# Nemo157/regex

Measured on AMD Instinct MI355X. Metric: haystack GB/s scanned + matches/s, batched bytes::Regex::find, 1/2/4/8 MI355X, higher is better.
Workload: dtype u8; 1 GPU; C2: find \d{4}-\d{2}-\d{2} over 1048576 x 4096 B haystacks per GPU; haystacks_per_gpu=1048576, haystack_bytes=4096, parallelism=dp1

## Files before the change

include/rure_amd.h:

```cpp
#ifndef RURE_AMD_H
#define RURE_AMD_H

#include <stdbool.h>
#include <stddef.h>
#include <stdint.h>

#ifdef __cplusplus
extern "C" {
#endif


typedef struct rure rure;
typedef struct rure_set rure_set;
typedef struct rure_options rure_options;
typedef struct rure_iter rure_iter;
typedef struct rure_error rure_error;
typedef struct rure_captures rure_captures;
typedef struct rure_iter_capture_names rure_iter_capture_names;

#define RURE_FLAG_CASEI (1 << 0)
#define RURE_FLAG_MULTI (1 << 1)
#define RURE_FLAG_DOTNL (1 << 2)
#define RURE_FLAG_SWAP_GREED (1 << 3)
#define RURE_FLAG_SPACE (1 << 4)
// ... 229 lines not shown
  RURE_AMD_PATH_ITER_CHUNKED = -21,
  RURE_AMD_PATH_ITER_WAVE = -22,
  RURE_AMD_PATH_REPLACE_CLASS = -23,
  RURE_AMD_PATH_REPLACE_HMAP = -24,
  RURE_AMD_PATH_ITER_SHADOW_GATED = -25,
  RURE_AMD_PATH_ITER_WAVE_SERVED = -27,
  RURE_AMD_PATH_CAPTURES_ITER = -28,
  RURE_AMD_PATH_REPLACE_EXPAND = -29
} rure_amd_path;
int rure_amd_last_fwd_path(void);
uint64_t rure_amd_last_iter_units(uint64_t *haystacks);
uint64_t rure_amd_last_long_units(uint64_t *haystacks, uint64_t *chunk);
uint64_t rure_amd_last_set_units(uint64_t *haystacks, uint64_t *chunk);
uint64_t rure_amd_last_lazy_long(uint64_t *haystacks, uint64_t *chunk, uint32_t *rounds, uint32_t *fell_back);
typedef struct rure_amd_tile_skip {
  int32_t eligible;
  int32_t m;
  int32_t anchor_a, anchor_b;
  int32_t used;
} rure_amd_tile_skip;
int rure_amd_tile_skip_info(rure *re, rure_amd_tile_skip *info);
int64_t rure_amd_tile_skip_simulate(rure *re, const uint8_t *hay, size_t len, uint32_t *states_skip,
                                    uint32_t *states_exact, uint8_t *dirty);
int rure_amd_debug_set(const char *spec);
int rure_amd_kernel_timer(int on);
double rure_amd_kernel_timer_read(uint64_t *launches);

#ifdef __cplusplus
}
#endif
#endif
```

regex_amd/__init__.py:

```python
import ctypes

from . import _native as N

__all__ = ["Regex", "RegexSet", "Error", "NoExpand", "NONE", "Path", "release_scratch"]

NONE = N.NONE
Path = N.Path


def _ser_lits(lits):
    out = bytearray()
    for v, cut in lits:
        out += bytes([1 if cut else 0]) + len(v).to_bytes(4, "little") + bytes(v)
    return bytes(out)


def _de_lits(buf):
    out, i = [], 0
    while i < len(buf):
        cut, n = buf[i] != 0, int.from_bytes(buf[i + 1:i + 5], "little")
        out.append((bytes(buf[i + 5:i + 5 + n]), cut))
        i += 5 + n
    return out

# ... 615 lines not shown
    def dfa_info(self, which=0):
        info = N.DfaInfo()
        rc = N.rure_amd_dfa_info_get(self._re, which, ctypes.byref(info))
        return {k: getattr(info, k) for k, _ in N.DfaInfo._fields_} if rc == N.OK else None

    def tile_skip_info(self):
        info = N.TileSkipInfo()
        rc = N.rure_amd_tile_skip_info(self._re, ctypes.byref(info))
        return {k: getattr(info, k) for k, _ in N.TileSkipInfo._fields_} if rc == N.OK else None

    def tile_skip_simulate(self, hay):
        import numpy as np
        hay = np.ascontiguousarray(np.frombuffer(bytes(hay), dtype=np.uint8))
        n = len(hay) // 128
        ss = np.zeros(max(n, 1), dtype=np.uint32)
        se = np.zeros(max(n, 1), dtype=np.uint32)
        d = np.zeros(max(n, 1), dtype=np.uint8)
        rc = N.rure_amd_tile_skip_simulate(self._re, hay.ctypes.data, len(hay), ss.ctypes.data, se.ctypes.data,
                                           d.ctypes.data)
        if rc < 0:
            return None
        return ss[:n], se[:n], d[:n]

    def first_bytes(self):
        buf = (ctypes.c_uint8 * 4)()
        n = N.rure_amd_first_byte_export(self._re, buf)
        return bytes(buf[:n]) if n > 0 else None

    def lex_table(self, ascii=False):
        import numpy as np
        if ascii:
            ex = lambda t, n, s: N.rure_amd_lex_ascii_export(self._re, 0, t, n, s)
        else:
            ex = lambda t, n, s: N.rure_amd_lex_export(self._re, t, n, s)
        n = ex(None, 0, None)
        if n <= 0:
            return None
        t = np.zeros(n, dtype=np.uint8)
        s0 = ctypes.c_uint32()
        ex(t.ctypes.data, n, ctypes.byref(s0))
        return t, s0.value

    def run_class(self, ascii=False):
        import numpy as np
        c = np.zeros(256, dtype=np.uint8)
        return c if N.rure_amd_run_class_export(self._re, 1 if ascii else 0, c.ctypes.data) == 1 else None
# ... 393 lines not shown
```

regex_amd/_native.py:

```python
import ctypes
import enum
import os

_HERE = os.path.dirname(os.path.abspath(__file__))
LIB_PATH = os.path.join(_HERE, "lib", "librure_amd.so")
if os.environ.get("RURE_AMD_LIB_AB"):
    LIB_PATH = os.path.join(_HERE, "lib", os.path.basename(os.environ["RURE_AMD_LIB_AB"]))

if not os.path.exists(LIB_PATH):
    raise ImportError(
        "regex_amd: native library %s is missing; build it with `make` or "
        "`python -c 'import __graft_entry__ as g; g.build()'`" % LIB_PATH)

try:
    import torch
except ImportError:
    pass

lib = ctypes.CDLL(LIB_PATH)

c_u8p = ctypes.POINTER(ctypes.c_uint8)
c_size = ctypes.c_size_t


# ... 167 lines not shown

def last_iter_units():
    n = ctypes.c_uint64(0)
    units = rure_amd_last_iter_units(ctypes.byref(n))
    return int(units), int(n.value)


rure_amd_last_long_units = _sig("rure_amd_last_long_units", ctypes.c_uint64, ctypes.POINTER(ctypes.c_uint64),
                                ctypes.POINTER(ctypes.c_uint64))


def last_long_units():
    n, c = ctypes.c_uint64(0), ctypes.c_uint64(0)
    units = rure_amd_last_long_units(ctypes.byref(n), ctypes.byref(c))
    return int(units), int(n.value), int(c.value)


class TileSkipInfo(ctypes.Structure):
    _fields_ = [(n, ctypes.c_int32) for n in ("eligible", "m", "anchor_a", "anchor_b", "used")]


rure_amd_tile_skip_info = _sig("rure_amd_tile_skip_info", ctypes.c_int, VP, ctypes.POINTER(TileSkipInfo))
rure_amd_tile_skip_simulate = _sig("rure_amd_tile_skip_simulate", ctypes.c_int64, VP, VP, c_size, VP, VP, VP)
rure_amd_last_set_units = _sig("rure_amd_last_set_units", ctypes.c_uint64, ctypes.POINTER(ctypes.c_uint64),
                               ctypes.POINTER(ctypes.c_uint64))
rure_amd_set_long_dfa_export = _sig("rure_amd_set_long_dfa_export", ctypes.c_int, VP, ctypes.POINTER(DfaInfo), VP, VP,
                                    VP, VP, VP, VP)
class LazyInfo(ctypes.Structure):
    _fields_ = [(k, ctypes.c_uint32) for k in ("states", "columns", "rows_built", "hot_rows", "rounds", "fell_back")]


rure_amd_set_lazy_export = _sig("rure_amd_set_lazy_export", ctypes.c_int, VP, ctypes.POINTER(LazyInfo), VP, VP, VP,
                                VP, VP, VP)
rure_amd_set_lazy_build = _sig("rure_amd_set_lazy_build", ctypes.c_int, VP, VP, c_size, c_size)
rure_amd_lazy_export = _sig("rure_amd_lazy_export", ctypes.c_int, VP, ctypes.POINTER(LazyInfo), VP, VP, VP, VP, VP)
rure_amd_lazy_build = _sig("rure_amd_lazy_build", ctypes.c_int, VP, VP, c_size, c_size)
rure_amd_lazy_strip_export = _sig("rure_amd_lazy_strip_export", ctypes.c_int, VP, VP)
rure_amd_set_lazy_strip_export = _sig("rure_amd_set_lazy_strip_export", ctypes.c_int, VP, VP, VP)
rure_amd_set_lazy_strip_build = _sig("rure_amd_set_lazy_strip_build", ctypes.c_int, VP, VP, c_size)
rure_amd_lazy_strip_build = _sig("rure_amd_lazy_strip_build", ctypes.c_int, VP, VP, c_size)
rure_amd_last_lazy_long = _sig("rure_amd_last_lazy_long", ctypes.c_uint64, ctypes.POINTER(ctypes.c_uint64),
                               ctypes.POINTER(ctypes.c_uint64), ctypes.POINTER(ctypes.c_uint32),
                               ctypes.POINTER(ctypes.c_uint32))
rure_amd_debug_set = _sig("rure_amd_debug_set", ctypes.c_int, ctypes.c_char_p)
rure_amd_first_byte_export = _sig("rure_amd_first_byte_export", ctypes.c_int, VP, VP)
rure_amd_lex_export = _sig("rure_amd_lex_export", ctypes.c_int64, VP, VP, c_size, VP)
# ... 46 lines not shown
```

regex_amd/csrc/capi.cpp:

```cpp
#include "runtime.hpp"
#include "host/chain_map.hpp"
#include "host/expand.hpp"

namespace {


void fill_prog_info(const Program &p, rure_amd_prog_info *info) {
  info->ninsts = (uint32_t)p.insts.size();
  info->start = p.start;
  info->nmatches = (uint32_t)p.matches.size();
  info->ncaptures = (uint32_t)p.capture_names.size();
  info->anchored_start = p.anchored_start;
  info->anchored_end = p.anchored_end;
  info->has_unicode_word_boundary = p.has_unicode_word_boundary;
  info->is_reverse = p.is_reverse;
  memcpy(info->byte_classes, p.byte_classes, 256);
}

int64_t export_prog(const Program &p, rure_amd_prog_info *info, rure_amd_inst *insts, size_t cap) {
  if (info) fill_prog_info(p, info);
  if (insts) {
    size_t n = std::min(cap, p.insts.size());
    for (size_t i = 0; i < n; ++i) {
      const Inst &in = p.insts[i];
// ... 1205 lines not shown
}
int rure_amd_tile_skip_info(rure *re, rure_amd_tile_skip *info) {
  if (!re || !info) return RURE_AMD_ERR_ARG;
  memset(info, 0, sizeof(*info));
  if (!build_regex(re) || !re->dfa_ok) return RURE_AMD_ERR_DFA;
  const TileSkip &k = re->tskip;
  info->eligible = k.ok ? 1 : 0;
  info->used = k.ok && k.use ? 1 : 0;
  info->m = (int32_t)k.m;
  info->anchor_a = k.ok ? (int32_t)k.pa : -1;
  info->anchor_b = k.ok ? (int32_t)k.pb : -1;
  return RURE_AMD_OK;
}

int64_t rure_amd_tile_skip_simulate(rure *re, const uint8_t *hay, size_t len, uint32_t *states_skip,
                                    uint32_t *states_exact, uint8_t *dirty) {
  if (!re || (!hay && len) || !states_skip || !states_exact || !dirty) return RURE_AMD_ERR_ARG;
  if (!build_regex(re) || !re->dfa_ok) return RURE_AMD_ERR_DFA;
  if (!re->tskip.ok) return RURE_AMD_ERR_ARG;
  return (int64_t)tile_skip_simulate(re->tskip, re->pf.lds.data(), re->pf.hot, re->pf.full.data(),
                                     (uint32_t)re->dfwd.n_match_end, hay, len, states_skip, states_exact, dirty);
}

int rure_amd_debug_set(const char *spec) { return rure_amd::knob_set(spec) ? RURE_AMD_OK : RURE_AMD_ERR_ARG; }



int64_t rure_amd_literals_syntax(const uint8_t *pattern, size_t length, uint32_t flags, int which, size_t limit_size,
                                 size_t limit_class, uint8_t *out, size_t cap) {
  Expr e;
  std::string err;
  if (!parse_regex(std::string((const char *)pattern, length), syntax_flags(flags), &e, &err)) return RURE_AMD_ERR_ARG;
  Literals l;
  l.limit_size = limit_size;
  l.limit_class = limit_class;
  if (which == 0) l.union_prefixes(e);
  else l.union_suffixes(e);
  std::string o;
  ser_lits(l.lits, &o);
  return put_out(o, out, cap);
}

int64_t rure_amd_literals_op(int op, const uint8_t *in, size_t in_len, uint8_t *out, size_t cap) {
  Literals l;
  if ((in_len && !in) || !de_lits(in, in_len, &l.lits)) return RURE_AMD_ERR_ARG;
  std::string o;
// ... 56 lines not shown
```

regex_amd/csrc/host/tile_skip.cpp:

```cpp
#include "tile_skip.hpp"

#include <algorithm>
#include <cstring>
#include <set>
#include <unordered_set>

#include "../kernels/dfa_scan.hpp"
#include "byte_freq.h"

namespace rure_amd {

namespace {

constexpr uint32_t kMaxPos = 16;

AsciiSet from_cranges(const std::vector<CRange> &r) {
  AsciiSet s;
  for (const CRange &x : r)
    for (uint32_t c = x.lo; c <= x.hi && c < 128; ++c) s.add(c);
  return s;
}

AsciiSet from_branges(const std::vector<BRange> &r) {
  AsciiSet s;
// ... 88 lines not shown
void tile_skip_analyse(const Expr &e, const uint8_t *lds, uint32_t hot, uint32_t ustart1, TileSkip *out) {
  TileSkip k;
  auto fail = [&](const std::string &w) { k.ok = false; k.why = w; *out = k; };
  if (!tile_skip_sequence(e, &k.seq, &k.why)) return fail(k.why);
  const uint32_t m = k.m = (uint32_t)k.seq.size();
  for (uint32_t b = 0; b < 128; ++b)
    for (uint32_t j = 0; j < m; ++j)
      if (k.seq[j].has(b)) k.sa[b] |= (uint16_t)(1u << j);
  struct Cand { double p; uint32_t pos; uint8_t lo, hi; };
  std::vector<Cand> cs;
  for (uint32_t j = 0; j < m; ++j) {
    uint8_t lo, hi;
    if (single_range(k.seq[j], &lo, &hi)) cs.push_back({range_freq(lo, hi), j, lo, hi});
  }
  if (cs.empty()) return fail("no position is a single byte range");
  std::stable_sort(cs.begin(), cs.end(), [](const Cand &x, const Cand &y) { return x.p < y.p; });
  Cand a = cs[0], b = cs.size() > 1 ? cs[1] : cs[0];
  if (a.pos > b.pos) std::swap(a, b);
  const double rate = 128.0 * a.p * (a.pos == b.pos ? 1.0 : b.p);
  if (rate >= 1.0) return fail("the anchors are too frequent");
  k.use = 64.0 * rate < 1.0;
  k.pa = a.pos; k.pb = b.pos;
  k.a_lo = a.lo; k.a_hi = a.hi; k.b_lo = b.lo; k.b_hi = b.hi;
  if (hot == 0 || hot > 63) return fail("no hot table of at most 63 rows");
  if (!ustart1) return fail("(S) the start state depends on the flags");
  k.s0 = ustart1 - 1;
  if (k.s0 >= hot) return fail("(S) the start state is not hot");
  auto step = [&](uint32_t s, uint32_t c) { return (uint32_t)lds[(size_t)s * kRow + c]; };
  const uint32_t fin = 1u << (m - 1);
  constexpr size_t kMaxProduct = 1 << 15;
  std::unordered_set<uint32_t> seen;
  std::vector<uint32_t> work;
  seen.insert(k.s0 << 17);
  work.push_back(k.s0 << 17);
  while (!work.empty()) {
    const uint32_t key = work.back(), s = key >> 17, D = (key >> 1) & 0xFFFFu, pc = key & 1u;
    work.pop_back();
    k.reach |= 1ull << s;
    for (uint32_t c = 0; c < 128; ++c) {
      const uint32_t D2 = ((D << 1) | 1u) & k.sa[c];
      const uint32_t comp = (D2 & fin) ? 1u : 0u;
      const uint32_t t = step(s, c);
      if (t == hot) {
        if (!comp && !pc) return fail("(A) the hot rows are left without a window of the sequence");
        continue;
      }
// ... 13 lines not shown
      for (uint32_t c = 0; c < 128; ++c) {
        const uint32_t p2 = step(pq.first, c);
        if (p2 == hot) continue;
        const uint32_t q2 = step(pq.second, c);
        if (q2 == hot) return fail("(B) the run from the start state leaves the hot rows first");
        next.insert({p2, q2});
      }
    level.swap(next);
  }
  for (const auto &pq : level)
    if (pq.first != pq.second) return fail("(B) the state after 16 bytes depends on the state before them");
  k.ok = true;
  *out = k;
}

void tile_skip_dev(const TileSkip &k, const uint16_t *sa, TileSkipDev *out) {
  TileSkipDev d{};
  const uint32_t rep = 0x01010101u;
  d.on = k.use ? 1 : 0; d.m = k.m; d.pa = k.pa; d.pb = k.pb; d.s0 = k.s0; d.reach = k.reach;
  d.gt_a = (0x7Fu - k.a_hi) * rep; d.lt_a = (0x7Fu + k.a_lo) * rep;
  d.gt_b = (0x7Fu - k.b_hi) * rep; d.lt_b = (0x7Fu + k.b_lo) * rep;
  d.eq_a = k.a_lo * rep; d.eq_b = k.b_lo * rep;
  d.single = k.a_lo == k.a_hi && k.b_lo == k.b_hi;
  d.sa = sa;
  *out = d;
}

namespace {

struct HostSrc {
  const uint8_t *p;
  uint4 row(int r) const {
    uint4 v;
    memcpy(&v, p + 16 * r, 16);
    return v;
  }
  uint32_t byte(uint32_t i) const { return p[i]; }
};

}

size_t tile_skip_simulate(const TileSkip &k, const uint8_t *lds, uint32_t hot, const uint16_t *full,
                          uint32_t n_match_end, const uint8_t *hay, size_t len, uint32_t *states_skip,
                          uint32_t *states_exact, uint8_t *dirty) {
  TileSkipDev kd;
  tile_skip_dev(k, k.sa, &kd);
// ... 12 lines not shown
    if (!done) {
      if (!d) {
        uint32_t c = k.s0;
        for (int j = 112; j < 128; ++j) c = lds[(size_t)c * kRow + p[j]];
        s = c;
        ln.prev_dirty = 0;
      } else {
        bool left = s >= hot;
        for (int j = 0; j < 128 && !done; ++j) {
          s = full[(size_t)s * 256 + p[j]];
          left = left || s >= hot;
          done = over(s);
        }
        ln.prev_dirty = (f & kSkipOwn) || left;
      }
    }
    states_skip[t] = s;
    for (int j = 0; j < 128 && !over(x); ++j) x = full[(size_t)x * 256 + p[j]];
    states_exact[t] = x;
  }
  return ntiles;
}

}
```

regex_amd/csrc/host/tile_skip.hpp:

```cpp
#pragma once
#include <cstdint>
#include <string>
#include <vector>

#include "syntax.hpp"

namespace rure_amd {

struct AsciiSet {
  uint64_t w[2] = {0, 0};
  bool has(uint32_t b) const { return (w[b >> 6] >> (b & 63)) & 1; }
  void add(uint32_t b) { w[b >> 6] |= 1ull << (b & 63); }
  bool empty() const { return !(w[0] | w[1]); }
};

struct TileSkip {
  bool ok = false;
  bool use = false;
  std::string why;
  uint32_t m = 0;
  std::vector<AsciiSet> seq;
  uint32_t pa = 0, pb = 0;
  uint8_t a_lo = 0, a_hi = 0, b_lo = 0, b_hi = 0;
  uint32_t s0 = 0;
  uint64_t reach = 0;
  uint16_t sa[128] = {0};
};

struct TileSkipDev;
void tile_skip_dev(const TileSkip &k, const uint16_t *sa, TileSkipDev *out);

bool tile_skip_sequence(const Expr &e, std::vector<AsciiSet> *seq, std::string *why);

void tile_skip_analyse(const Expr &e, const uint8_t *lds, uint32_t hot, uint32_t ustart1, TileSkip *out);

size_t tile_skip_simulate(const TileSkip &k, const uint8_t *lds, uint32_t hot, const uint16_t *full,
                          uint32_t n_match_end, const uint8_t *hay, size_t len, uint32_t *states_skip,
                          uint32_t *states_exact, uint8_t *dirty);

}
```

regex_amd/csrc/kernels/dfa_scan.hip:

```cpp
#include <hip/hip_runtime.h>
#include <stdint.h>

#include <algorithm>
#include <cstdlib>
#include <mutex>
#include <vector>

#include "dfa_device.hpp"

namespace rure_amd {

__device__ __forceinline__ void note_quit(uint32_t *flag) {
  if (flag) atomicOr(flag, 1u);
}

template <int MODE>
__device__ __forceinline__ void finish_lane(const LaneState &L, const RevDfaDev &r, const uint8_t *base,
                                            uint64_t len, uint64_t lo, uint64_t h, void *out, uint32_t *qf,
                                            const uint8_t *rlds = nullptr) {
  if (L.quit) note_quit(qf);
  if (MODE == MODE_ISMATCH) {
    ((uint8_t *)out)[h] = L.quit ? 2 : (L.last != NONE ? 1 : 0);
    return;
  }
// ... 176 lines not shown
  const bool strided = b.offs == nullptr;
  if (!strided && b.defer)
    return mode == MODE_FIND ? launch_lit_find_m<MODE_FIND, false, true>(b, f, out, st, grid)
                             : launch_lit_find_m<MODE_ISMATCH, false, true>(b, f, out, st, grid);
  if (mode == MODE_FIND)
    return strided ? launch_lit_find_m<MODE_FIND, true>(b, f, out, st, grid)
                   : launch_lit_find_m<MODE_FIND, false>(b, f, out, st, grid);
  return strided ? launch_lit_find_m<MODE_ISMATCH, true>(b, f, out, st, grid)
                 : launch_lit_find_m<MODE_ISMATCH, false>(b, f, out, st, grid);
}

static constexpr int kTileTab = 64 * kRow + 256;
static constexpr int kTileTabSmall = 16 * kRow + 96;

struct TileSkipSrc {
  const uint4 *buf;
  int lane, sw;
  __device__ __forceinline__ uint4 row(int r) const { return buf[lane * 8 + (r ^ sw)]; }
  __device__ __forceinline__ uint32_t byte(uint32_t p) const {
    return ((const uint8_t *)buf)[(lane * 8 + ((p >> 4) ^ sw)) * 16 + (p & 15)];
  }
};

template <int MODE, int TAB, int STRIDE, bool SKIP = false>
__global__ __launch_bounds__(256, SKIP && TAB == kTileTabSmall ? 4 : 1) void dfa_fwd_tile_kernel(BatchDev bt,
                                                                                                 FwdDfaDev f,
                                                                                                 RevDfaDev r,
                                                                                                 void *out,
                                                                                                 uint64_t gscatter) {
  static_assert(!SKIP || STRIDE == 1, "the skip rule reads the byte table");
  __shared__ __attribute__((aligned(16))) uint8_t tab[TAB];
  __shared__ uint16_t sa[SKIP ? 128 : 1];
  if (SKIP && threadIdx.x < 128) sa[threadIdx.x] = f.skip.sa[threadIdx.x];
  const uint8_t *img = STRIDE == 1 ? f.lds_image : f.lds_image_s;
  const uint32_t img_bytes = STRIDE == 1 ? f.lds_bytes : f.lds_bytes_s;
  __shared__ __attribute__((aligned(16))) uint4 stage[4][64 * 8];
  for (uint32_t i = threadIdx.x * 16; i < img_bytes; i += blockDim.x * 16)
    *(uint4 *)(tab + i) = *(const uint4 *)(img + i);
  __syncthreads();
  const uint16_t *tab16 = (const uint16_t *)(tab + 1024);
  const int lane = threadIdx.x & 63, w = threadIdx.x >> 6;
  uint4 *buf = stage[w];
  const uint64_t L = bt.length, S = bt.stride, n = bt.count;
  const uint64_t L128 = L & ~(uint64_t)127;
  const uint64_t nwaves = (uint64_t)gridDim.x * 4;
  const int src_h = lane >> 3, src_seg = lane & 7;
  const uint64_t ngroups = (n + 63) / 64;
  for (uint64_t gi = (uint64_t)blockIdx.x * 4 + w; gi < ngroups; gi += nwaves) {
// ... 3 lines not shown
    const uint8_t *base = bt.hay + (valid ? h : 0) * S;
    LaneState L_;
    L_.last = NONE;
    L_.quit = false;
    L_.done = !valid;
    L_.s = valid ? f.start[fwd_flag_index(base, L, 0)] : f.dead;
    if (L_.s >= f.n_normal) L_.done = true;
    L_.fast = STRIDE > 1 && !L_.done && L_.s < f.hot_s;
    L_.t = L_.fast ? L_.s * f.P : 0;
    TileSkipLane K_{};
    uint64_t hh0 = g * 64 + src_h;
    const uint8_t *src0 = bt.hay + (hh0 < n ? hh0 : n - 1) * S + 16 * src_seg;
    const uint64_t kstep = 8 * S;
    const uint64_t klast = (n - 1) * S + 16 * src_seg;
    uint4 n0, n1, n2, n3, n4, n5, n6, n7;
    uint64_t at = 0;
#define RURE_SRC(k) ((g * 64 + 8 * (k) + src_h < n) ? src0 + (k) * kstep : bt.hay + klast)
#define RURE_LOAD_TILE(a)                                                          \
  n0 = *(const uint4 *)(RURE_SRC(0) + (a)); n1 = *(const uint4 *)(RURE_SRC(1) + (a));  \
  n2 = *(const uint4 *)(RURE_SRC(2) + (a)); n3 = *(const uint4 *)(RURE_SRC(3) + (a));  \
  n4 = *(const uint4 *)(RURE_SRC(4) + (a)); n5 = *(const uint4 *)(RURE_SRC(5) + (a));  \
  n6 = *(const uint4 *)(RURE_SRC(6) + (a)); n7 = *(const uint4 *)(RURE_SRC(7) + (a));
#define RURE_STAGE(k, v) buf[(8 * (k) + src_h) * 8 + (src_seg ^ (((8 * (k) + src_h) >> 1) & 7))] = (v);
    if (L128) { RURE_LOAD_TILE(0) }
    const int sw = (lane >> 1) & 7;
    for (; at < L128; at += 128) {
      if (!__any(!L_.done)) break;
      RURE_STAGE(0, n0) RURE_STAGE(1, n1) RURE_STAGE(2, n2) RURE_STAGE(3, n3)
      RURE_STAGE(4, n4) RURE_STAGE(5, n5) RURE_STAGE(6, n6) RURE_STAGE(7, n7)
      wave_lds_sync();
      const uint64_t an = (at + 128 < L128) ? at + 128 : at;
      if (!SKIP) { RURE_LOAD_TILE(an) }
      uint4 cur = buf[lane * 8 + sw];
      bool walk = true;
      uint32_t pdirty = 0;
      if (SKIP) {
        pdirty = tile_skip_dirty(f.skip, sa, TileSkipSrc{buf, lane, sw}, K_, L_.s);
        __builtin_amdgcn_fence(__ATOMIC_ACQUIRE, "wavefront");
        RURE_LOAD_TILE(an)
        if (!__any(!L_.done && (pdirty & kSkipDirty))) {
          const uint4 v = buf[lane * 8 + (7 ^ sw)];
          uint32_t t = f.skip.s0;
          t = fast4(t, v.x, tab);
          t = fast4(t, v.y, tab);
          t = fast4(t, v.z, tab);
          t = fast4(t, v.w, tab);
          if (!L_.done) L_.s = t;
          K_.prev_dirty = 0;
          walk = false;
        }
      }
      if (!walk) {
      } else if (STRIDE == 1) {
        const uint32_t hot = f.hot;
        uint32_t t = (L_.done || L_.s >= hot) ? hot : L_.s;
        uint32_t bad = (L_.done || L_.s < hot) ? 8u : 0u;
        uint32_t sbad = L_.s;
#pragma unroll
        for (int m = 0; m < 8; ++m) {
          const uint4 nx = buf[lane * 8 + ((m + 1 < 8 ? m + 1 : 7) ^ sw)];
          const uint32_t t0 = t;
          t = fast4(t, cur.x, tab);
          t = fast4(t, cur.y, tab);
          t = fast4(t, cur.z, tab);
          t = fast4(t, cur.w, tab);
          const bool hit = (t == hot) & (t0 != hot);
          bad = hit ? (uint32_t)m : bad;
          sbad = hit ? t0 : sbad;
          cur = nx;
        }
        if (bad < 8) {
          L_.s = sbad;
#pragma unroll 1
          for (uint32_t m = bad; m < 8 && !L_.done; ++m) {
            const uint4 v = buf[lane * 8 + (m ^ sw)];
            const uint32_t words[4] = {v.x, v.y, v.z, v.w};
#pragma unroll 1
            for (int j = 0; j < 16 && !L_.done; ++j)
              step1<MODE>(L_, f, tab, (words[j >> 2] >> ((j & 3) * 8)) & 0xFF, at + 16 * m + j);
          }
        } else if (!L_.done) {
          L_.s = t;
        }
        if (SKIP) K_.prev_dirty = (pdirty & kSkipOwn) || bad < 8;
      } else {
#pragma unroll 1
        for (int m = 0; m < 8; ++m) {
          uint4 nx = buf[lane * 8 + ((m + 1 < 8 ? m + 1 : 7) ^ sw)];
          if (!L_.done) chunk16s<MODE, STRIDE>(L_, f, tab, tab16, cur, at + 16 * m);
          cur = nx;
        }
      }
      wave_lds_sync();
    }
#undef RURE_LOAD_TILE
#undef RURE_SRC
#undef RURE_STAGE
    if (valid) {
      if (STRIDE > 1 && L_.fast) { L_.s = L_.t / f.P; L_.fast = false; }
      at = L128;
      while (!L_.done && at < L) {
        if (STRIDE == 1) step1<MODE>(L_, f, tab, base[at], at);
        else careful_step<MODE>(L_, f, base[at], at);
        ++at;
      }
      if (!L_.done && f.eof[L_.s]) L_.last = L;
      finish_lane<MODE>(L_, r, base, L, 0, h, out, bt.quit_flag);
    }
  }
}

template <bool STRIDED>
__global__ __launch_bounds__(256) void dfa_set_kernel(BatchDev bt, SetDfaDev f, uint64_t *out) {
  extern __shared__ __attribute__((aligned(16))) uint8_t lds[];
  for (uint32_t i = threadIdx.x * 16; i < f.lds_bytes; i += blockDim.x * 16)
    *(uint4 *)(lds + i) = *(const uint4 *)(f.lds_image + i);
  __syncthreads();
// ... 529 lines not shown
    hipLaunchKernelGGL((dfa_fwd_kernel<MODE, false, false, true>), dim3(grid), dim3(256), f.lds_bytes, st, b, f, r,
                       out);
  else
    hipLaunchKernelGGL((dfa_fwd_kernel<MODE, STRIDED, false>), dim3(grid), dim3(256), f.lds_bytes, st, b, f, r, out);
  return hipGetLastError();
}


template <int MODE, int STRIDE>
static hipError_t launch_tile_s(const BatchDev &b, const FwdDfaDev &f, const RevDfaDev &r, void *out, hipStream_t st,
                                int grid) {
  const uint32_t bytes = STRIDE == 1 ? f.lds_bytes : f.lds_bytes_s;
  static_assert(RURE_AMD_PATH_TILE1 == 1 && RURE_AMD_PATH_TILE2 == 2 && RURE_AMD_PATH_TILE4 == 4,
                "the tile paths are numbered by their stride");
  constexpr rure_amd_path kPath =
      STRIDE == 4 ? RURE_AMD_PATH_TILE4 : STRIDE == 2 ? RURE_AMD_PATH_TILE2 : RURE_AMD_PATH_TILE1;
  note_fwd_path(kPath);
  const uint64_t ngroups = (b.count + 63) / 64;
  uint64_t mul = 40503;
  auto gcd = [](uint64_t a, uint64_t c) { while (c) { uint64_t t = a % c; a = c; c = t; } return a; };
  while (ngroups > 1 && gcd(mul, ngroups) != 1) mul += 2;
  if (ngroups <= 1) mul = 0;
  if (STRIDE == 1 && f.skip.on && knob(Knob::TileSkip) != 0) {
    if (bytes <= (uint32_t)kTileTabSmall)
      hipLaunchKernelGGL((dfa_fwd_tile_kernel<MODE, kTileTabSmall, 1, true>), dim3(grid), dim3(256), 0, st, b, f, r,
                         out, mul);
    else
      hipLaunchKernelGGL((dfa_fwd_tile_kernel<MODE, kTileTab, 1, true>), dim3(grid), dim3(256), 0, st, b, f, r, out,
                         mul);
    return hipGetLastError();
  }
  if (bytes <= (uint32_t)kTileTabSmall)
    hipLaunchKernelGGL((dfa_fwd_tile_kernel<MODE, kTileTabSmall, STRIDE>), dim3(grid), dim3(256), 0, st, b, f, r, out,
                       mul);
  else
    hipLaunchKernelGGL((dfa_fwd_tile_kernel<MODE, kTileTab, STRIDE>), dim3(grid), dim3(256), 0, st, b, f, r, out, mul);
  return hipGetLastError();
}

template <int MODE>
static hipError_t launch_tile(const BatchDev &b, const FwdDfaDev &f, const RevDfaDev &r, void *out, hipStream_t st,
                              int grid) {
  const bool latency_bound = b.count <= (uint64_t)f.cus * 16 * 64 / 2;
  if (latency_bound && f.stride == 4 && f.lds_bytes_s <= (uint32_t)kTileTab) return launch_tile_s<MODE, 4>(b, f, r, out, st, grid);
  if (latency_bound && f.stride == 2 && f.lds_bytes_s <= (uint32_t)kTileTab) return launch_tile_s<MODE, 2>(b, f, r, out, st, grid);
  return launch_tile_s<MODE, 1>(b, f, r, out, st, grid);
}

bool tile_path_ok(const BatchDev &b, const FwdDfaDev &f) {
  return b.offs == nullptr && b.start == 0 && (b.stride % 16) == 0 && (((uintptr_t)b.hay) & 15) == 0 &&
         b.length <= b.stride && b.length >= 128 &&
         f.lds_bytes <= (uint32_t)kTileTab;
// ... 45 lines not shown
```

regex_amd/csrc/kernels/tile_skip_device.hpp:

```cpp
#pragma once
#include <hip/hip_runtime.h>
#include <stdint.h>

namespace rure_amd {

struct TileSkipDev {
  uint32_t on;
  uint32_t m;
  uint32_t pa, pb;
  uint32_t gt_a, lt_a, gt_b, lt_b;
  uint32_t eq_a, eq_b;
  uint32_t single;
  uint32_t s0;
  uint64_t reach;
  const uint16_t *sa;
};

struct TileSkipLane {
  uint32_t c0, c1, c2, c3;
  uint32_t cflags;
  uint32_t prev_dirty;
};

__host__ __device__ __forceinline__ uint32_t skip_gather4(uint32_t x, uint32_t acc, int sh) {
#if defined(__HIP_DEVICE_COMPILE__)
  return __builtin_amdgcn_udot4(x, 0x08040201u << sh, acc, false);
#else
  return acc + (((((x >> 7) * 0x00204081u) >> 21) & 0xFu) << (sh + 7));
#endif
}

template <bool SINGLE>
__host__ __device__ __forceinline__ uint32_t skip_miss(uint32_t w, uint32_t eq, uint32_t gt, uint32_t lt) {
  return (SINGLE ? (w ^ eq) + 0x7F7F7F7Fu : ((w + gt) | (lt - w))) & 0x80808080u;
}

template <bool SINGLE>
__host__ __device__ __forceinline__ uint32_t skip_row_misses(const uint4 &v, uint32_t eq, uint32_t gt, uint32_t lt) {
// ... 48 lines not shown
        uint32_t ok = 1;
        for (uint32_t j = 0; j < k.m; ++j) {
          const int p = q + (int)j;
          const uint32_t b = p < 0 ? skip_carry_byte(o0, o1, o2, o3, (uint32_t)(p + 16)) : src.byte((uint32_t)(p < 0 ? 0 : p));
          ok &= (uint32_t)sa[b & 127] >> j;
        }
        dirty = ok & 1;
      }
    }
  }
  return dirty ? (kSkipDirty | kSkipOwn) : (ln.prev_dirty ? kSkipDirty : 0u);
}

template <class Src>
__host__ __device__ __forceinline__ uint32_t tile_skip_dirty(const TileSkipDev &k, const uint16_t *sa, const Src &src,
                                                         TileSkipLane &ln, uint32_t s) {
  const bool same = k.gt_a == k.gt_b && k.lt_a == k.lt_b;
  if (k.single) return same ? tile_skip_dirty_as<true, true>(k, sa, src, ln, s)
                            : tile_skip_dirty_as<true, false>(k, sa, src, ln, s);
  return same ? tile_skip_dirty_as<false, true>(k, sa, src, ln, s)
              : tile_skip_dirty_as<false, false>(k, sa, src, ln, s);
}

}
```

Measured before the change: 5528 GB/s.

## Add wave-cooperative tile prescan with confirm anchors to skip clean tiles

Adds a prescan mode to the tile-skip DFA kernel. Raw global tile loads are checked in registers: anchor and up to two confirm-position byte-class flags are combined across lanes with DPP shifts. Only suspect tiles are staged to LDS and walked; clean tiles are skipped and the state is rebuilt lazily from the last 16 bytes. This is meant to cut LDS staging, syncs and dirty checks for rare-match patterns like dates, at the cost of extra register pressure, changed occupancy bounds and more complex carry logic across tiles. A host simulator is added for validation.

Measured after the change: 4027 GB/s. 27.1% lower.

```diff
diff --git a/include/rure_amd.h b/include/rure_amd.h
--- a/include/rure_amd.h
+++ b/include/rure_amd.h
@@ -275,6 +275,8 @@
 int rure_amd_tile_skip_info(rure *re, rure_amd_tile_skip *info);
 int64_t rure_amd_tile_skip_simulate(rure *re, const uint8_t *hay, size_t len, uint32_t *states_skip,
                                     uint32_t *states_exact, uint8_t *dirty);
+int64_t rure_amd_tile_prescan_simulate(rure *re, const uint8_t *hay, size_t len, uint8_t *suspect, uint32_t *states,
+                                       int64_t *ends);
 int rure_amd_debug_set(const char *spec);
 int rure_amd_kernel_timer(int on);
 double rure_amd_kernel_timer_read(uint64_t *launches);
diff --git a/regex_amd/__init__.py b/regex_amd/__init__.py
--- a/regex_amd/__init__.py
+++ b/regex_amd/__init__.py
@@ -661,6 +661,20 @@
             return None
         return ss[:n], se[:n], d[:n]
 
+    def tile_prescan_simulate(self, hays):
+        import numpy as np
+        hays = np.ascontiguousarray(hays, dtype=np.uint8)
+        assert hays.ndim == 2 and hays.shape[0] == 64 and hays.shape[1] >= 128, hays.shape
+        n = hays.shape[1] // 128
+        sus = np.zeros(n, dtype=np.uint8)
+        st = np.zeros(64, dtype=np.uint32)
+        en = np.zeros(64, dtype=np.int64)
+        rc = N.rure_amd_tile_prescan_simulate(self._re, hays.ctypes.data, hays.shape[1], sus.ctypes.data,
+                                              st.ctypes.data, en.ctypes.data)
+        if rc < 0:
+            return None
+        return sus, st, en
+
     def first_bytes(self):
         buf = (ctypes.c_uint8 * 4)()
         n = N.rure_amd_first_byte_export(self._re, buf)
diff --git a/regex_amd/_native.py b/regex_amd/_native.py
--- a/regex_amd/_native.py
+++ b/regex_amd/_native.py
@@ -213,6 +213,7 @@
 
 rure_amd_tile_skip_info = _sig("rure_amd_tile_skip_info", ctypes.c_int, VP, ctypes.POINTER(TileSkipInfo))
 rure_amd_tile_skip_simulate = _sig("rure_amd_tile_skip_simulate", ctypes.c_int64, VP, VP, c_size, VP, VP, VP)
+rure_amd_tile_prescan_simulate = _sig("rure_amd_tile_prescan_simulate", ctypes.c_int64, VP, VP, c_size, VP, VP, VP)
 rure_amd_last_set_units = _sig("rure_amd_last_set_units", ctypes.c_uint64, ctypes.POINTER(ctypes.c_uint64),
                                ctypes.POINTER(ctypes.c_uint64))
 rure_amd_set_long_dfa_export = _sig("rure_amd_set_long_dfa_export", ctypes.c_int, VP, ctypes.POINTER(DfaInfo), VP, VP,
diff --git a/regex_amd/csrc/capi.cpp b/regex_amd/csrc/capi.cpp
--- a/regex_amd/csrc/capi.cpp
+++ b/regex_amd/csrc/capi.cpp
@@ -1251,6 +1251,16 @@
                                      (uint32_t)re->dfwd.n_match_end, hay, len, states_skip, states_exact, dirty);
 }
 
+int64_t rure_amd_tile_prescan_simulate(rure *re, const uint8_t *hay, size_t len, uint8_t *suspect, uint32_t *states,
+                                       int64_t *ends) {
+  if (!re || !hay || len < 128 || !suspect || !states || !ends) return RURE_AMD_ERR_ARG;
+  if (!build_regex(re) || !re->dfa_ok) return RURE_AMD_ERR_DFA;
+  if (!re->tskip.ok) return RURE_AMD_ERR_ARG;
+  return (int64_t)tile_prescan_simulate(re->tskip, re->pf.lds.data(), re->pf.hot, re->pf.full.data(),
+                                        re->pf.eof.data(), (uint32_t)re->dfwd.n_normal,
+                                        (uint32_t)re->dfwd.n_match_end, hay, len, suspect, states, ends);
+}
+
 int rure_amd_debug_set(const char *spec) { return rure_amd::knob_set(spec) ? RURE_AMD_OK : RURE_AMD_ERR_ARG; }
 
 
diff --git a/regex_amd/csrc/host/tile_skip.cpp b/regex_amd/csrc/host/tile_skip.cpp
--- a/regex_amd/csrc/host/tile_skip.cpp
+++ b/regex_amd/csrc/host/tile_skip.cpp
@@ -134,6 +134,15 @@
   k.use = 64.0 * rate < 1.0;
   k.pa = a.pos; k.pb = b.pos;
   k.a_lo = a.lo; k.a_hi = a.hi; k.b_lo = b.lo; k.b_hi = b.hi;
+  auto dist = [&](const Cand &x) { return x.pos > b.pos ? x.pos - b.pos : b.pos - x.pos; };
+  std::stable_sort(cs.begin(), cs.end(), [&](const Cand &x, const Cand &y) {
+    return x.p != y.p ? x.p < y.p : dist(x) < dist(y);
+  });
+  for (const Cand &c : cs)
+    if (c.pos != a.pos && c.pos != b.pos && c.p < 0.5 && k.nconf < 2) {
+      k.c_pos[k.nconf] = c.pos; k.c_lo[k.nconf] = c.lo; k.c_hi[k.nconf] = c.hi;
+      ++k.nconf;
+    }
   if (hot == 0 || hot > 63) return fail("no hot table of at most 63 rows");
   if (!ustart1) return fail("(S) the start state depends on the flags");
   k.s0 = ustart1 - 1;
@@ -193,6 +202,11 @@
   d.gt_b = (0x7Fu - k.b_hi) * rep; d.lt_b = (0x7Fu + k.b_lo) * rep;
   d.eq_a = k.a_lo * rep; d.eq_b = k.b_lo * rep;
   d.single = k.a_lo == k.a_hi && k.b_lo == k.b_hi;
+  d.nconf = k.nconf;
+  for (uint32_t i = 0; i < k.nconf; ++i) {
+    d.cd[i] = (int32_t)k.c_pos[i] - (int32_t)k.pb;
+    d.gt_c[i] = (0x7Fu - k.c_hi[i]) * rep; d.lt_c[i] = (0x7Fu + k.c_lo[i]) * rep;
+  }
   d.sa = sa;
   *out = d;
 }
@@ -251,4 +265,146 @@
   return ntiles;
 }
 
-}
+namespace {
+
+bool prescan_wave(const TileSkipDev &kd, const uint4 (*T)[8], TilePrescan *P, uint64_t done) {
+  const bool one = kd.single && kd.eq_a == kd.eq_b;
+  uint32_t sus[64], pend[64], ca[64][4];
+  for (int l = 0; l < 64; ++l) {
+    sus[l] = P[l].pend;
+    pend[l] = 0;
+    ca[l][0] = ca[l][1] = ca[l][2] = ca[l][3] = 0;
+  }
+  for (int i = 0; i < 8; ++i) {
+    uint32_t fab[64], c[64], fc[64], c2[64];
+    bool any = false;
+    for (int l = 0; l < 64; ++l)
+      fab[l] = one ? skip_row_flags<true, true>(kd, T[l][i]) : skip_row_flags<false, false>(kd, T[l][i]);
+    for (int l = 0; l < 64; ++l) {
+      const PrescanHostWave w{fab, l};
+      uint32_t carry;
+      c[l] = prescan_cand(kd, w, fab[l], (uint32_t)l & 7, (P[l].ca[i >> 1] >> (16 * (i & 1))) & 0xFFFFu, &carry);
+      ca[l][i >> 1] |= carry << (16 * (i & 1));
+      any = any || c[l] != 0;
+    }
+    for (uint32_t j = 0; any && j < kd.nconf; ++j) {
+      for (int l = 0; l < 64; ++l) fc[l] = prescan_conf_flags(kd, j, T[l][i]);
+      for (int l = 0; l < 64; ++l) c2[l] = prescan_confirm(kd, PrescanHostWave{fc, l}, j, c[l], fc[l], (uint32_t)l & 7);
+      memcpy(c, c2, sizeof(c));
+    }
+    for (int l = 0; l < 64; ++l) {
+      const uint4 &v = T[l][i];
+      const uint32_t late = prescan_late(kd, c[l], (uint32_t)l & 7);
+      const uint32_t high = (v.x | v.y | v.z | v.w) & 0x80808080u;
+      sus[l] |= (high | (c[l] ^ late)) ? 1u << i : 0u;
+      pend[l] |= late ? 1u << i : 0u;
+    }
+  }
+  bool suspect = false;
+  for (int l = 0; l < 64; ++l) {
+    memcpy(P[l].ca, ca[l], sizeof(ca[l]));
+    P[l].pend = pend[l];
+    suspect = suspect || (sus[l] & prescan_live8(done, (uint32_t)l >> 3)) != 0;
+  }
+  return suspect;
+}
+
+}
+
+size_t tile_prescan_simulate(const TileSkip &k, const uint8_t *lds, uint32_t hot, const uint16_t *full,
+                             const uint8_t *eof, uint32_t n_normal, uint32_t n_match_end, const uint8_t *hay,
+                             size_t len, uint8_t *suspect, uint32_t *states, int64_t *ends) {
+  TileSkipDev kd;
+  tile_skip_dev(k, k.sa, &kd);
+  kd.on = 1;
+  const size_t ntiles = len / 128;
+  struct Lane {
+    uint32_t s = 0;
+    int64_t last = -1;
+    bool done = false;
+    TileSkipLane K{};
+  } ln[64];
+  TilePrescan P[64];
+  memset(P, 0, sizeof(P));
+  for (Lane &x : ln) {
+    x.s = k.s0;
+    x.done = x.s >= n_normal;
+  }
+  auto chain16 = [&](const uint8_t *p) {
+    uint32_t c = k.s0;
+    for (int j = 0; j < 16; ++j) c = lds[(size_t)c * kRow + p[j]];
+    return c;
+  };
+  auto enter = [&](Lane &x, uint32_t b, uint64_t pos) {
+    x.s = full[(size_t)x.s * 256 + b];
+    if (x.s >= n_normal) {
+      if (x.s < n_match_end) x.last = (int64_t)pos;
+      else x.done = true;
+    }
+  };
+  bool stale = false;
+  std::vector<uint4> regs(64 * 8);
+  uint4(*T)[8] = (uint4(*)[8])regs.data();
+  for (size_t t = 0; t < ntiles; ++t) {
+    const size_t at = 128 * t;
+    uint64_t done = 0;
+    for (int l = 0; l < 64; ++l) done |= (uint64_t)ln[l].done << l;
+    suspect[t] = 0;
+    if (!~done) continue;
+    for (int l = 0; l < 64; ++l)
+      for (int i = 0; i < 8; ++i) memcpy(&T[l][i], hay + (size_t)(8 * i + (l >> 3)) * len + at + 16 * (l & 7), 16);
+    bool sus = prescan_wave(kd, T, P, done);
+    for (const Lane &x : ln) {
+      const bool lost = !stale && (x.s >= 64 || !((kd.reach >> x.s) & 1));
+      sus = sus || (!x.done && (x.K.prev_dirty || lost));
+    }
+    suspect[t] = sus ? 1 : 0;
+    if (!sus) {
+      stale = true;
+      continue;
+    }
+    bool any = false;
+    uint32_t pd[64];
+    for (int l = 0; l < 64; ++l) {
+      Lane &x = ln[l];
+      const uint8_t *p = hay + (size_t)l * len + at;
+      if (at) {
+        if (stale && !x.done) x.s = chain16(p - 16);
+        uint4 c;
+        memcpy(&c, p - 16, 16);
+        x.K.c0 = c.x; x.K.c1 = c.y; x.K.c2 = c.z; x.K.c3 = c.w;
+        x.K.cflags = skip_row_flags(kd, c);
+      }
+      pd[l] = tile_skip_dirty(kd, k.sa, HostSrc{p}, x.K, x.s);
+      any = any || (!x.done && (pd[l] & kSkipDirty));
+    }
+    stale = false;
+    for (int l = 0; l < 64; ++l) {
+      Lane &x = ln[l];
+      const uint8_t *p = hay + (size_t)l * len + at;
+      if (!any) {
+        if (!x.done) x.s = chain16(p + 112);
+        x.K.prev_dirty = 0;
+        continue;
+      }
+      bool left = !x.done && x.s >= hot;
+      for (int j = 0; j < 128 && !x.done; ++j) {
+        enter(x, p[j], at + j);
+        left = left || x.s >= hot;
+      }
+      x.K.prev_dirty = (pd[l] & kSkipOwn) || left;
+    }
+  }
+  for (int l = 0; l < 64; ++l) {
+    Lane &x = ln[l];
+    const uint8_t *p = hay + (size_t)l * len;
+    if (stale && !x.done) x.s = chain16(p + 128 * ntiles - 16);
+    states[l] = x.s;
+    for (size_t at = 128 * ntiles; at < len && !x.done; ++at) enter(x, p[at], at);
+    if (!x.done && eof[x.s]) x.last = (int64_t)len;
+    ends[l] = x.last;
+  }
+  return ntiles;
+}
+
+}
diff --git a/regex_amd/csrc/host/tile_skip.hpp b/regex_amd/csrc/host/tile_skip.hpp
--- a/regex_amd/csrc/host/tile_skip.hpp
+++ b/regex_amd/csrc/host/tile_skip.hpp
@@ -22,6 +22,9 @@
   std::vector<AsciiSet> seq;
   uint32_t pa = 0, pb = 0;
   uint8_t a_lo = 0, a_hi = 0, b_lo = 0, b_hi = 0;
+  uint32_t nconf = 0;
+  uint32_t c_pos[2] = {0, 0};
+  uint8_t c_lo[2] = {0, 0}, c_hi[2] = {0, 0};
   uint32_t s0 = 0;
   uint64_t reach = 0;
   uint16_t sa[128] = {0};
@@ -38,4 +41,8 @@
                           uint32_t n_match_end, const uint8_t *hay, size_t len, uint32_t *states_skip,
                           uint32_t *states_exact, uint8_t *dirty);
 
+size_t tile_prescan_simulate(const TileSkip &k, const uint8_t *lds, uint32_t hot, const uint16_t *full,
+                             const uint8_t *eof, uint32_t n_normal, uint32_t n_match_end, const uint8_t *hay,
+                             size_t len, uint8_t *suspect, uint32_t *states, int64_t *ends);
+
 }
diff --git a/regex_amd/csrc/kernels/dfa_scan.hip b/regex_amd/csrc/kernels/dfa_scan.hip
--- a/regex_amd/csrc/kernels/dfa_scan.hip
+++ b/regex_amd/csrc/kernels/dfa_scan.hip
@@ -222,8 +222,43 @@
   }
 };
 
-template <int MODE, int TAB, int STRIDE, bool SKIP = false>
-__global__ __launch_bounds__(256, SKIP && TAB == kTileTabSmall ? 4 : 1) void dfa_fwd_tile_kernel(BatchDev bt,
+template <bool SINGLE, bool SAME>
+__device__ __forceinline__ bool tile_prescan_as(const TileSkipDev &k, const uint4 (&T)[8], uint32_t seg, uint32_t h,
+                                                TilePrescan &P, uint64_t done) {
+  const PrescanWave w;
+  uint32_t sus = P.pend, pend = 0, ca[4] = {0, 0, 0, 0};
+#pragma unroll
+  for (int i = 0; i < 8; ++i) {
+    const uint32_t fab = skip_row_flags<SINGLE, SAME>(k, T[i]);
+    uint32_t carry;
+    uint32_t c = prescan_cand(k, w, fab, seg, (P.ca[i >> 1] >> (16 * (i & 1))) & 0xFFFFu, &carry);
+    ca[i >> 1] |= carry << (16 * (i & 1));
+    if (__any(c != 0)) {
+      if (k.nconf > 0) c = prescan_confirm(k, w, 0, c, prescan_conf_flags(k, 0, T[i]), seg);
+      if (k.nconf > 1) c = prescan_confirm(k, w, 1, c, prescan_conf_flags(k, 1, T[i]), seg);
+    }
+    const uint32_t late = prescan_late(k, c, seg);
+    const uint32_t high = (T[i].x | T[i].y | T[i].z | T[i].w) & 0x80808080u;
+    sus |= (high | (c ^ late)) ? 1u << i : 0u;
+    pend |= late ? 1u << i : 0u;
+  }
+  P.ca[0] = ca[0]; P.ca[1] = ca[1]; P.ca[2] = ca[2]; P.ca[3] = ca[3];
+  P.pend = pend;
+  if (!__any(sus != 0)) return false;
+  return __any((sus & prescan_live8(done, h)) != 0);
+}
+
+__device__ __forceinline__ bool tile_prescan(const TileSkipDev &k, const uint4 (&T)[8], uint32_t seg, uint32_t h,
+                                             TilePrescan &P, uint64_t done) {
+  if (k.single && k.eq_a == k.eq_b) return tile_prescan_as<true, true>(k, T, seg, h, P, done);
+  return tile_prescan_as<false, false>(k, T, seg, h, P, done);
+}
+
+#ifndef RURE_TILE_PRESCAN_WAVES
+#define RURE_TILE_PRESCAN_WAVES 4
+#endif
+template <int MODE, int TAB, int STRIDE, int SKIP = 0>
+__global__ __launch_bounds__(256, !SKIP ? 1 : TAB != kTileTabSmall ? (SKIP == 2 ? 3 : 1) : SKIP == 2 ? RURE_TILE_PRESCAN_WAVES : 4) void dfa_fwd_tile_kernel(BatchDev bt,
                                                                                                  FwdDfaDev f,
                                                                                                  RevDfaDev r,
                                                                                                  void *out,
@@ -273,77 +308,144 @@
   n4 = *(const uint4 *)(RURE_SRC(4) + (a)); n5 = *(const uint4 *)(RURE_SRC(5) + (a));  \
   n6 = *(const uint4 *)(RURE_SRC(6) + (a)); n7 = *(const uint4 *)(RURE_SRC(7) + (a));
 #define RURE_STAGE(k, v) buf[(8 * (k) + src_h) * 8 + (src_seg ^ (((8 * (k) + src_h) >> 1) & 7))] = (v);
-    if (L128) { RURE_LOAD_TILE(0) }
     const int sw = (lane >> 1) & 7;
-    for (; at < L128; at += 128) {
-      if (!__any(!L_.done)) break;
-      RURE_STAGE(0, n0) RURE_STAGE(1, n1) RURE_STAGE(2, n2) RURE_STAGE(3, n3)
-      RURE_STAGE(4, n4) RURE_STAGE(5, n5) RURE_STAGE(6, n6) RURE_STAGE(7, n7)
-      wave_lds_sync();
-      const uint64_t an = (at + 128 < L128) ? at + 128 : at;
-      if (!SKIP) { RURE_LOAD_TILE(an) }
-      uint4 cur = buf[lane * 8 + sw];
-      bool walk = true;
-      uint32_t pdirty = 0;
-      if (SKIP) {
-        pdirty = tile_skip_dirty(f.skip, sa, TileSkipSrc{buf, lane, sw}, K_, L_.s);
-        __builtin_amdgcn_fence(__ATOMIC_ACQUIRE, "wavefront");
-        RURE_LOAD_TILE(an)
-        if (!__any(!L_.done && (pdirty & kSkipDirty))) {
-          const uint4 v = buf[lane * 8 + (7 ^ sw)];
-          uint32_t t = f.skip.s0;
-          t = fast4(t, v.x, tab);
-          t = fast4(t, v.y, tab);
-          t = fast4(t, v.z, tab);
-          t = fast4(t, v.w, tab);
-          if (!L_.done) L_.s = t;
-          K_.prev_dirty = 0;
-          walk = false;
+#define RURE_TILE_STAGED(PREFETCH)                                                          \
+  {                                                                                         \
+    uint4 cur = buf[lane * 8 + sw];                                                         \
+    bool walk = true;                                                                       \
+    uint32_t pdirty = 0;                                                                    \
+    if (SKIP) {                                                                             \
+      pdirty = tile_skip_dirty(f.skip, sa, TileSkipSrc{buf, lane, sw}, K_, L_.s);           \
+      __builtin_amdgcn_fence(__ATOMIC_ACQUIRE, "wavefront");                                \
+      PREFETCH                                                                              \
+      if (!__any(!L_.done && (pdirty & kSkipDirty))) {                                      \
+        const uint4 v = buf[lane * 8 + (7 ^ sw)];                                           \
+        uint32_t t = f.skip.s0;                                                             \
+        t = fast4(t, v.x, tab);                                                             \
+        t = fast4(t, v.y, tab);                                                             \
+        t = fast4(t, v.z, tab);                                                             \
+        t = fast4(t, v.w, tab);                                                             \
+        if (!L_.done) L_.s = t;                                                             \
+        K_.prev_dirty = 0;                                                                  \
+        walk = false;                                                                       \
+      }                                                                                     \
+    }                                                                                       \
+    if (!walk) {                                                                            \
+    } else if (STRIDE == 1) {                                                               \
+      const uint32_t hot = f.hot;                                                           \
+      uint32_t t = (L_.done || L_.s >= hot) ? hot : L_.s;                                   \
+      uint32_t bad = (L_.done || L_.s < hot) ? 8u : 0u;    \
+      uint32_t sbad = L_.s;                                                                 \
+      _Pragma("unroll") for (int m = 0; m < 8; ++m) {                                       \
+        const uint4 nx = buf[lane * 8 + ((m + 1 < 8 ? m + 1 : 7) ^ sw)];                    \
+        const uint32_t t0 = t;                                                              \
+        t = fast4(t, cur.x, tab);                                                           \
+        t = fast4(t, cur.y, tab);                                                           \
+        t = fast4(t, cur.z, tab);                                                           \
+        t = fast4(t, cur.w, tab);                                                           \
+        const bool hit = (t == hot) & (t0 != hot);                                          \
+        bad = hit ? (uint32_t)m : bad;                                                      \
+        sbad = hit ? t0 : sbad;                                                             \
+        cur = nx;                                                                           \
+      }                                                                                     \
+      if (bad < 8) {                                                                        \
+        L_.s = sbad;                                                                        \
+        _Pragma("unroll 1") for (uint32_t m = bad; m < 8 && !L_.done; ++m) {                \
+          const uint4 v = buf[lane * 8 + (m ^ sw)];                                         \
+          const uint32_t words[4] = {v.x, v.y, v.z, v.w};                                   \
+          _Pragma("unroll 1") for (int j = 0; j < 16 && !L_.done; ++j)                      \
+              step1<MODE>(L_, f, tab, (words[j >> 2] >> ((j & 3) * 8)) & 0xFF, at + 16 * m + j); \
+        }                                                                                   \
+      } else if (!L_.done) {                                                                \
+        L_.s = t;                                                                           \
+      }                                                                                     \
+      if (SKIP) K_.prev_dirty = (pdirty & kSkipOwn) || bad < 8;                             \
+    } else {                                                                                \
+      _Pragma("unroll 1") for (int m = 0; m < 8; ++m) {                                     \
+        uint4 nx = buf[lane * 8 + ((m + 1 < 8 ? m + 1 : 7) ^ sw)];                          \
+        if (!L_.done) chunk16s<MODE, STRIDE>(L_, f, tab, tab16, cur, at + 16 * m);          \
+        cur = nx;                                                                           \
+      }                                                                                     \
+    }                                                                                       \
+  }
+    if constexpr (SKIP == 2) {
+      uint4 A[8], B[8];
+      TilePrescan P_{};
+      bool stale = false;
+      const uint64_t g0 = ((uint64_t)__builtin_amdgcn_readfirstlane((uint32_t)(g >> 32)) << 32) |
+                          __builtin_amdgcn_readfirstlane((uint32_t)g);
+      const uint8_t *gbase = bt.hay + g0 * 64 * S;
+      uint32_t off[8];
+#pragma unroll
+      for (int k_ = 0; k_ < 8; ++k_) {
+        const uint64_t row = g0 * 64 + 8 * k_ + src_h;
+        off[k_] = (uint32_t)((row < n ? row : n - 1) - g0 * 64) * (uint32_t)S + 16 * src_seg;
+      }
+#define RURE_LOAD_SET(T, a)                                                          \
+  _Pragma("unroll") for (int k_ = 0; k_ < 8; ++k_) T[k_] = *(const uint4 *)(gbase + (a) + off[k_]);
+      if (L128) { RURE_LOAD_SET(A, 0) }
+      for (; at < L128; at += 128) {
+        const uint64_t done = __ballot(L_.done);
+        if (!~done) break;
+        const uint64_t an = (at + 128 < L128) ? at + 128 : at;
+        RURE_LOAD_SET(B, an)
+        bool sus = tile_prescan(f.skip, A, (uint32_t)src_seg, (uint32_t)src_h, P_, done);
+        const bool lost = !stale && (L_.s >= 64 || !((f.skip.reach >> L_.s) & 1));
+        sus = __any(!L_.done && (K_.prev_dirty || lost)) || sus;
+        if (!sus) {
+          stale = true;
+        } else {
+          if (at) {
+            uint4 c;
+            if (stale) {
+              c = *(const uint4 *)(base + at - 16);
+              uint32_t t = f.skip.s0;
+              t = fast4(t, c.x, tab);
+              t = fast4(t, c.y, tab);
+              t = fast4(t, c.z, tab);
+              t = fast4(t, c.w, tab);
+              if (!L_.done) L_.s = t;
+            } else {
+              c = buf[lane * 8 + (7 ^ sw)];
+              wave_lds_sync();
+            }
+            K_.c0 = c.x; K_.c1 = c.y; K_.c2 = c.z; K_.c3 = c.w;
+            K_.cflags = skip_row_flags(f.skip, c);
+          }
+          stale = false;
+#pragma unroll
+          for (int k_ = 0; k_ < 8; ++k_) { RURE_STAGE(k_, A[k_]) }
+          wave_lds_sync();
+          RURE_TILE_STAGED(RURE_LOAD_SET(B, an))
+          wave_lds_sync();
         }
+#pragma unroll
+        for (int k_ = 0; k_ < 8; ++k_) A[k_] = B[k_];
       }
-      if (!walk) {
-      } else if (STRIDE == 1) {
-        const uint32_t hot = f.hot;
-        uint32_t t = (L_.done || L_.s >= hot) ? hot : L_.s;
-        uint32_t bad = (L_.done || L_.s < hot) ? 8u : 0u;
-        uint32_t sbad = L_.s;
-#pragma unroll
-        for (int m = 0; m < 8; ++m) {
-          const uint4 nx = buf[lane * 8 + ((m + 1 < 8 ? m + 1 : 7) ^ sw)];
-          const uint32_t t0 = t;
-          t = fast4(t, cur.x, tab);
-          t = fast4(t, cur.y, tab);
-          t = fast4(t, cur.z, tab);
-          t = fast4(t, cur.w, tab);
-          const bool hit = (t == hot) & (t0 != hot);
-          bad = hit ? (uint32_t)m : bad;
-          sbad = hit ? t0 : sbad;
-          cur = nx;
-        }
-        if (bad < 8) {
-          L_.s = sbad;
-#pragma unroll 1
-          for (uint32_t m = bad; m < 8 && !L_.done; ++m) {
-            const uint4 v = buf[lane * 8 + (m ^ sw)];
-            const uint32_t words[4] = {v.x, v.y, v.z, v.w};
-#pragma unroll 1
-            for (int j = 0; j < 16 && !L_.done; ++j)
-              step1<MODE>(L_, f, tab, (words[j >> 2] >> ((j & 3) * 8)) & 0xFF, at + 16 * m + j);
-          }
-        } else if (!L_.done) {
-          L_.s = t;
-        }
-        if (SKIP) K_.prev_dirty = (pdirty & kSkipOwn) || bad < 8;
-      } else {
-#pragma unroll 1
-        for (int m = 0; m < 8; ++m) {
-          uint4 nx = buf[lane * 8 + ((m + 1 < 8 ? m + 1 : 7) ^ sw)];
-          if (!L_.done) chunk16s<MODE, STRIDE>(L_, f, tab, tab16, cur, at + 16 * m);
-          cur = nx;
-        }
+#undef RURE_LOAD_SET
+      if (stale && !L_.done) {
+        const uint4 c = *(const uint4 *)(base + L128 - 16);
+        uint32_t t = f.skip.s0;
+        t = fast4(t, c.x, tab);
+        t = fast4(t, c.y, tab);
+        t = fast4(t, c.z, tab);
+        t = fast4(t, c.w, tab);
+        L_.s = t;
       }
-      wave_lds_sync();
-    }
+    } else {
+      if (L128) { RURE_LOAD_TILE(0) }
+      for (; at < L128; at += 128) {
+        if (!__any(!L_.done)) break;
+        RURE_STAGE(0, n0) RURE_STAGE(1, n1) RURE_STAGE(2, n2) RURE_STAGE(3, n3)
+        RURE_STAGE(4, n4) RURE_STAGE(5, n5) RURE_STAGE(6, n6) RURE_STAGE(7, n7)
+        wave_lds_sync();
+        const uint64_t an = (at + 128 < L128) ? at + 128 : at;
+        if (!SKIP) { RURE_LOAD_TILE(an) }
+        RURE_TILE_STAGED(RURE_LOAD_TILE(an))
+        wave_lds_sync();
+      }
+    }
+#undef RURE_TILE_STAGED
 #undef RURE_LOAD_TILE
 #undef RURE_SRC
 #undef RURE_STAGE
@@ -919,12 +1021,22 @@
   while (ngroups > 1 && gcd(mul, ngroups) != 1) mul += 2;
   if (ngroups <= 1) mul = 0;
   if (STRIDE == 1 && f.skip.on && knob(Knob::TileSkip) != 0) {
-    if (bytes <= (uint32_t)kTileTabSmall)
-      hipLaunchKernelGGL((dfa_fwd_tile_kernel<MODE, kTileTabSmall, 1, true>), dim3(grid), dim3(256), 0, st, b, f, r,
-                         out, mul);
-    else
-      hipLaunchKernelGGL((dfa_fwd_tile_kernel<MODE, kTileTab, 1, true>), dim3(grid), dim3(256), 0, st, b, f, r, out,
-                         mul);
+    const bool pre = knob(Knob::TileSkip) != 1 && b.stride < (1ull << 25);
+    if (bytes <= (uint32_t)kTileTabSmall) {
+      if (pre)
+        hipLaunchKernelGGL((dfa_fwd_tile_kernel<MODE, kTileTabSmall, 1, 2>), dim3(grid), dim3(256), 0, st, b, f, r,
+                           out, mul);
+      else
+        hipLaunchKernelGGL((dfa_fwd_tile_kernel<MODE, kTileTabSmall, 1, 1>), dim3(grid), dim3(256), 0, st, b, f, r,
+                           out, mul);
+    } else {
+      if (pre)
+        hipLaunchKernelGGL((dfa_fwd_tile_kernel<MODE, kTileTab, 1, 2>), dim3(grid), dim3(256), 0, st, b, f, r, out,
+                           mul);
+      else
+        hipLaunchKernelGGL((dfa_fwd_tile_kernel<MODE, kTileTab, 1, 1>), dim3(grid), dim3(256), 0, st, b, f, r, out,
+                           mul);
+    }
     return hipGetLastError();
   }
   if (bytes <= (uint32_t)kTileTabSmall)
diff --git a/regex_amd/csrc/kernels/tile_skip_device.hpp b/regex_amd/csrc/kernels/tile_skip_device.hpp
--- a/regex_amd/csrc/kernels/tile_skip_device.hpp
+++ b/regex_amd/csrc/kernels/tile_skip_device.hpp
@@ -14,6 +14,9 @@
   uint32_t s0;
   uint64_t reach;
   const uint16_t *sa;
+  uint32_t nconf;
+  int32_t cd[2];
+  uint32_t gt_c[2], lt_c[2];
 };
 
 struct TileSkipLane {
@@ -108,4 +111,74 @@
               : tile_skip_dirty_as<false, false>(k, sa, src, ln, s);
 }
 
+
+template <bool SINGLE, bool SAME>
+__host__ __device__ __forceinline__ uint32_t skip_row_flags(const TileSkipDev &k, const uint4 &v) {
+  const uint32_t fa = ~skip_row_misses<SINGLE>(v, k.eq_a, k.gt_a, k.lt_a) & 0xFFFFu;
+  const uint32_t fb = SAME ? fa : (~skip_row_misses<SINGLE>(v, k.eq_b, k.gt_b, k.lt_b) & 0xFFFFu);
+  return fa | (fb << 16);
 }
+
+__host__ __device__ __forceinline__ uint32_t skip_row_flags(const TileSkipDev &k, const uint4 &v) {
+  const bool same = k.gt_a == k.gt_b && k.lt_a == k.lt_b;
+  if (k.single) return same ? skip_row_flags<true, true>(k, v) : skip_row_flags<true, false>(k, v);
+  return same ? skip_row_flags<false, true>(k, v) : skip_row_flags<false, false>(k, v);
+}
+
+struct TilePrescan {
+  uint32_t ca[4];
+  uint32_t pend;
+};
+
+struct PrescanWave {
+  __device__ __forceinline__ uint32_t below1(uint32_t x) const {
+    return (uint32_t)__builtin_amdgcn_update_dpp(0, (int)x, 0x111, 0xF, 0xF, true);
+  }
+  __device__ __forceinline__ uint32_t above1(uint32_t x) const {
+    return (uint32_t)__builtin_amdgcn_update_dpp(0, (int)x, 0x101, 0xF, 0xF, true);
+  }
+  __device__ __forceinline__ uint32_t above7(uint32_t x) const {
+    return (uint32_t)__builtin_amdgcn_update_dpp(0, (int)x, 0x107, 0xF, 0xF, true);
+  }
+};
+struct PrescanHostWave {
+  const uint32_t *all;
+  int lane;
+  uint32_t below1(uint32_t) const { return (lane & 15) ? all[lane - 1] : 0u; }
+  uint32_t above1(uint32_t) const { return (lane & 15) != 15 ? all[lane + 1] : 0u; }
+  uint32_t above7(uint32_t) const { return (lane & 15) + 7 < 16 ? all[lane + 7] : 0u; }
+};
+
+template <class W>
+__host__ __device__ __forceinline__ uint32_t prescan_cand(const TileSkipDev &k, const W &w, uint32_t fab, uint32_t seg,
+                                                         uint32_t carried, uint32_t *carry) {
+  const uint32_t below = w.below1(fab) & 0xFFFFu;
+  *carry = w.above7(fab) & 0xFFFFu;
+  const uint32_t before = seg ? below : carried;
+  return (fab >> 16) & ((((fab & 0xFFFFu) << 16) | before) >> (16 - (k.pb - k.pa))) & 0xFFFFu;
+}
+
+__host__ __device__ __forceinline__ uint32_t prescan_conf_flags(const TileSkipDev &k, uint32_t i, const uint4 &v) {
+  return ~skip_row_misses<false>(v, 0, k.gt_c[i], k.lt_c[i]) & 0xFFFFu;
+}
+
+template <class W>
+__host__ __device__ __forceinline__ uint32_t prescan_confirm(const TileSkipDev &k, const W &w, uint32_t i, uint32_t c,
+                                                            uint32_t fc, uint32_t seg) {
+  const uint32_t below = w.below1(fc), above = w.above1(fc);
+  const uint32_t lo = seg ? below : 0xFFFFu, hi = seg != 7 ? above : 0xFFFFu;
+  const uint64_t win = (uint64_t)lo | ((uint64_t)fc << 16) | ((uint64_t)hi << 32);
+  return c & (uint32_t)(win >> (16 + k.cd[i])) & 0xFFFFu;
+}
+
+__host__ __device__ __forceinline__ uint32_t prescan_late(const TileSkipDev &k, uint32_t c, uint32_t seg) {
+  return seg == 7 ? c & ~(0xFFFFu >> (k.m - 1 - k.pb)) : 0u;
+}
+
+__host__ __device__ __forceinline__ uint32_t prescan_live8(uint64_t done, uint32_t h) {
+  const uint64_t x = ~done >> h;
+  const uint32_t lo = (uint32_t)x & 0x01010101u, hi = (uint32_t)(x >> 32) & 0x01010101u;
+  return skip_gather4(hi << 7, skip_gather4(lo << 7, 0, 0), 4) >> 7;
+}
+
+}
```
